# neuromodulation/PyPARRM

Measured on NVIDIA B200. Metric: filter_data channel-samples/sec, higher is better.
Workload: dtype f64

## Files before the change

### pyparrm_b200/_native.py

```python

from __future__ import annotations

import ctypes
import os
from ctypes import POINTER, c_char_p, c_double, c_int, c_int32, c_int64, c_size_t, c_void_p

LIB_NAME = "libparrm_b200.so"
LIB_PATH = os.path.join(os.path.dirname(os.path.abspath(__file__)), LIB_NAME)

F64, F32, I16, I32 = 0, 1, 2, 3
DIR_BOTH, DIR_PAST, DIR_FUTURE = 0, 1, 2
DIRECTIONS = {"both": DIR_BOTH, "past": DIR_PAST, "future": DIR_FUTURE}
MAX_BANDWIDTH = 23
NM_STATE_BYTES = 88
ABI_VERSION = 8
PLAN_AUTO, PLAN_GATHER, PLAN_COMB = 0, 1, 2
KERNEL_AUTO, KERNEL_GATHER, KERNEL_SPECIALISED = 0, 1, 3


class FilterOptions(ctypes.Structure):

    _fields_ = [
        ("kernel", c_int32),
        ("steps_per_chunk", c_int32),
# ... 112 lines not shown
            f"{LIB_NAME} is not built (expected {LIB_PATH}). Build it with "
            "`python -c 'import __graft_entry__ as g; g.build()'` or "
            "`pyparrm_b200/csrc/build.sh`. pyparrm_b200 has no CPU fallback."
        )
    lib = ctypes.CDLL(LIB_PATH)
    for name, (restype, argtypes) in SIGNATURES.items():
        fn = getattr(lib, name)
        fn.restype = restype
        fn.argtypes = argtypes
    if lib.parrm_abi_version() != ABI_VERSION:
        raise ImportError(
            f"{LIB_NAME} has ABI version {lib.parrm_abi_version()}, expected {ABI_VERSION}; rebuild it."
        )
    return lib


lib = _load()


def last_error() -> str:
    msg = lib.parrm_last_error()
    return msg.decode("utf-8", "replace") if msg else ""


def check(status: int, what: str) -> None:
    if status != 0:
        raise RuntimeError(f"{what} failed (status {status}): {last_error()}")


def filter_last_kernel() -> str:
    name = lib.parrm_filter_last_kernel()
    return name.decode() if name else ""


def device_count() -> int:
    return int(lib.parrm_device_count())


def plan_filter(taps, dtype: int = F64, strategy: int = PLAN_AUTO):
    import numpy as np

    taps = np.ascontiguousarray(taps, dtype=np.int32)
    nbytes = lib.parrm_filter_plan_bytes(taps.ctypes.data, int(taps.shape[0]))
    plan = np.zeros(nbytes, dtype=np.uint8)
    check(lib.parrm_filter_plan(taps.ctypes.data, int(taps.shape[0]), dtype, strategy,
                                plan.ctypes.data, nbytes), "parrm_filter_plan")
    info = np.zeros(16, dtype=np.int32)
    terms = np.zeros(256, dtype=np.int32)
    check(lib.parrm_filter_plan_info(plan.ctypes.data, info.ctypes.data, terms.ctypes.data, 256),
          "parrm_filter_plan_info")
    kind, stride, n_kinds, w0, w1, b0, b1, n_plus, n_minus, centre, cost = (int(v) for v in info[:11])
    cuts = np.cumsum([0, b0, b1, n_plus, n_minus])
    parts = [terms[cuts[i]:cuts[i + 1]].copy() for i in range(4)]
    desc = {
        "kind": kind, "stride": stride, "windows": [w0, w1][:n_kinds],
        "boxes": parts[:2][:n_kinds], "plus": parts[2], "minus": parts[3],
        "centre": centre, "cost": cost / 1000.0, "n_taps": int(info[11]),
    }
    return plan, desc
```

### pyparrm_b200/csrc/filter_comb_e.cuh

```cuda
#pragma once

#ifdef __CUDACC_RTC__
typedef signed char int8_t;
typedef int int32_t;
typedef unsigned int uint32_t;
typedef long long int64_t;
typedef unsigned long long uint64_t;
typedef unsigned long long uintptr_t;
#else
#include <stdint.h>
#endif

#ifndef PE_D
#define PE_T double
#define PE_D 200
#define PE_NK 2
#define PE_M0 20
#define PE_M1 10
#define PE_NB0 7
#define PE_NB1 2
#define PE_OFF0 -1969, -1954, -1923, -1877, -1846, -1831, -1800
#define PE_OFF1 -1908, 108
#define PE_NPLUS 1
#define PE_PLUS -2000
#define PE_NMINUS 0
#define PE_MINUS 0
#define PE_CENTRE -1
#define PE_U 10
#define PE_PF 2
#define PE_NTAPS 160
#define PE_WLO -2000
#define PE_WHI 2000
#define PE_BACK 108
#define PE_FWD 2000
#define PE_CTAS 2
#endif
#ifndef PE_VARIANT
#define PE_VARIANT 0
#endif

namespace parrm_e {

typedef PE_T T;
typedef double T2;
constexpr int D = PE_D;
constexpr int NK = PE_NK;
constexpr int M0 = PE_M0;
constexpr int M1 = PE_M1;
constexpr int NB0 = PE_NB0;
constexpr int NB1 = PE_NB1;
constexpr int NPLUS = PE_NPLUS;
constexpr int NMINUS = PE_NMINUS;
constexpr int CENTRE = PE_CENTRE;
constexpr int U = PE_U;
constexpr int PF = PE_PF;
constexpr int NTAPS = PE_NTAPS;
constexpr int WLO = PE_WLO;
constexpr int WHI = PE_WHI;
constexpr int BACK = PE_BACK;
constexpr int FWD = PE_FWD;
constexpr int ES = int(sizeof(T));
constexpr int VEC = 16 / ES;
constexpr int CH = U * D;
constexpr int HB = (BACK + CH - 1) / CH;
constexpr int HF = (FWD + CH - 1) / CH;
constexpr int MIR = HB + HF;
constexpr int Q = HB + HF + 1 + PF;
constexpr int GPB = (M0 + U - 1) / U;
constexpr int B = GPB * U;
constexpr int NPG = GPB;
constexpr int NW = (D + 31) / 32;
constexpr int NT = NW * 32 + 32;
constexpr int BAR_BYTES = ((2 * Q * 8 + 127) / 128) * 128;
constexpr int SMEM_BYTES = BAR_BYTES + (Q + MIR) * CH * ES;
static_assert((CH * ES) % 16 == 0, "chunk must be a whole number of 16-byte units");
static_assert(M0 >= M1 && M0 >= 1, "box lengths ordered");

__host__ __device__ constexpr int off0(int b) {
  constexpr int t[NB0 > 0 ? NB0 : 1] = {PE_OFF0};
  return t[b];
}
__host__ __device__ constexpr int off1(int b) {
  constexpr int t[NB1 > 0 ? NB1 : 1] = {PE_OFF1};
  return t[b];
}
__host__ __device__ constexpr int plus_tap(int i) {
  constexpr int t[NPLUS > 0 ? NPLUS : 1] = {PE_PLUS};
  return t[i];
}
__host__ __device__ constexpr int minus_tap(int i) {
  constexpr int t[NMINUS > 0 ? NMINUS : 1] = {PE_MINUS};
  return t[i];
}

struct Args {
  const T* x;
  T* out;
  const int32_t* taps;
  const int32_t* count;
  const T2* recip;
  int64_t ld_x, x_t0, n_x;
  int64_t ld_out, t0, n_out;
  int64_t n_total;
  int64_t total_groups;
  int32_t groups_per_chan;
  int32_t edge_start;
  int32_t edge_total;
  int32_t pad;
  unsigned long long* timeline;
  T neg_inv_n;
  T t_max;
};

__device__ __forceinline__ uint32_t smem_u32(const void* p) {
  return static_cast<uint32_t>(__cvta_generic_to_shared(p));
}
__device__ __forceinline__ void mbar_init(uint64_t* bar, uint32_t count) {
  asm volatile("mbarrier.init.shared::cta.b64 [%0], %1;" ::"r"(smem_u32(bar)), "r"(count));
}
__device__ __forceinline__ void mbar_expect_tx(uint64_t* bar, uint32_t bytes) {
  asm volatile("mbarrier.arrive.expect_tx.shared::cta.b64 _, [%0], %1;" ::"r"(smem_u32(bar)),
               "r"(bytes)
               : "memory");
}
__device__ __forceinline__ void mbar_arrive(uint64_t* bar) {
  asm volatile("mbarrier.arrive.shared::cta.b64 _, [%0];" ::"r"(smem_u32(bar)) : "memory");
}
__device__ __forceinline__ void mbar_wait(uint32_t bar, uint32_t parity) {
  asm volatile(
      "{\n"
      ".reg .pred p;\n"
      "WAIT_%=:\n"
      "mbarrier.try_wait.parity.shared::cta.b64 p, [%0], %1;\n"
      "@p bra DONE_%=;\n"
      "bra WAIT_%=;\n"
      "DONE_%=:\n"
      "}\n" ::"r"(bar),
      "r"(parity)
      : "memory");
}
__device__ __forceinline__ void bulk_g2s(void* dst_smem, const void* src_gmem, uint32_t bytes,
                                         uint64_t* bar) {
  asm volatile(
      "cp.async.bulk.shared::cluster.global.mbarrier::complete_tx::bytes [%0], [%1], %2, [%3];" ::
          "r"(smem_u32(dst_smem)),
      "l"(src_gmem), "r"(bytes), "r"(smem_u32(bar))
// ... 15 lines not shown
  const int n_in = count[v1 - (WLO - 1)] - count[v2 - (WLO - 1)];
  T y = xc - tot * T(recip[n_in]);
  if (n_in == 0) y = T(0);
  return y;
}

__device__ __noinline__ T direct_value(const int32_t* __restrict__ taps,
                                       const T2* __restrict__ recip, int64_t n_total, T t_max,
                                       const T* __restrict__ xrow, int64_t t, int64_t lo_valid,
                                       int64_t hi_valid) {
  T acc = T(0);
  int n_in = 0;
  for (int k = 0; k < NTAPS; ++k) {
    const int64_t g = t - taps[k];
    if (g < 0 || g >= n_total) continue;
    ++n_in;
    if (g >= lo_valid && g < hi_valid) acc += xrow[g];
  }
  if (n_in == 0) return T(0);
  const T y = xrow[t] - acc * T(recip[n_in]);
  return fabs(y) <= t_max ? y : T(0);
}

struct Walk {
  int pb;
  int rslot;
  int fslot;
  uint32_t fphase;
};

__device__ __forceinline__ void group_begin(Walk& w, uint32_t bars) {
  mbar_wait(bars + w.fslot * 8, w.fphase);
  if (++w.fslot == Q) {
    w.fslot = 0;
    w.fphase ^= 1u;
  }
}
__device__ __forceinline__ void group_end(Walk& w, uint32_t bars, int lane, unsigned wmask) {
  __syncwarp(wmask);
  if (lane == 0) {
    asm volatile("mbarrier.arrive.shared::cta.b64 _, [%0];" ::"r"(bars + (Q + w.rslot) * 8)
                 : "memory");
  }
  w.pb += CH * ES;
  if (++w.rslot == Q) {
    w.rslot = 0;
    w.pb -= Q * CH * ES;
  }
}

struct Rings {
  T r0[B];
  T r1[NK > 1 ? B : 1];
  T S0, S1;
};

__device__ __forceinline__ T ring_sum0(const Rings& r, int s) {
  T a = r.r0[s];
#pragma unroll
  for (int i = 1; i < M0; ++i) a += r.r0[(s + B - i) % B];
  return a;
}
__device__ __forceinline__ T ring_sum1(const Rings& r, int s) {
  if (NK < 2) return T(0);
  T a = r.r1[s];
#pragma unroll
  for (int i = 1; i < M1; ++i) a += r.r1[(s + B - i) % B];
  return a;
}

template <bool FAST>
__device__ __forceinline__ int run_block(Rings& r, Walk& w, const Args& a,
                                         const unsigned char* const smem, uint32_t bars,
                                         int lane, unsigned wmask, int c, T* const orow,
                                         int& bad_lo, int& bad_hi, int64_t Tb, int g,
                                         int n_groups) {
  const T neg_inv_n = a.neg_inv_n;
  const T t_max = a.t_max;
  T* const op = orow + Tb + c;
  int done = 0;
#pragma unroll
  for (int gi = 0; gi < GPB; ++gi) {
    if (!FAST && g + gi >= n_groups) break;
    group_begin(w, bars);
    int mode = 1;
    if (!FAST) {
      const int64_t Tn = Tb + int64_t(gi) * CH;
      const bool interior = (Tn - WHI >= 0) && (Tn + CH - WLO <= a.n_total);
      const bool all_out = (Tn >= a.t0) && (Tn + CH <= a.t0 + a.n_out);
      mode = (g + gi < NPG) ? 0 : ((interior && all_out) ? 1 : 2);
    }
    const unsigned char* const p = smem + w.pb;
#pragma unroll
    for (int js = 0; js < U; ++js) {
      const int s = gi * U + js;
      auto ld = [&](int off) {
        return *reinterpret_cast<const T*>(p + (HB * CH + js * D - off) * ES);
      };
      r.S0 -= r.r0[(s + B - M0) % B];
      if (NK > 1) r.S1 -= r.r1[(s + B - M1) % B];
      T e0 = ld(off0(0));
      if (NB0 > 1) {
        T e0b = ld(off0(1));
#pragma unroll
        for (int b = 2; b < NB0; ++b) {
          if (b & 1) e0b += ld(off0(b)); else e0 += ld(off0(b));
        }
        e0 += e0b;
      }
      r.r0[s] = e0;
      r.S0 += e0;
      T tot = r.S0;
      if (NK > 1) {
        T e1 = ld(off1(0));
        if (NB1 > 1) {
          T e1b = ld(off1(1));
#pragma unroll
          for (int b = 2; b < NB1; ++b) {
            if (b & 1) e1b += ld(off1(b)); else e1 += ld(off1(b));
          }
          e1 += e1b;
        }
        r.r1[s] = e1;
        r.S1 += e1;
        tot += r.S1;
      }
      T single = T(0);
      if (NPLUS > 0) {
        single = ld(plus_tap(0));
#pragma unroll
        for (int i = 1; i < NPLUS; ++i) single += ld(plus_tap(i));
      }
#pragma unroll
      for (int i = 0; i < NMINUS; ++i) single -= ld(minus_tap(i));
      const T xc = ld(0);
      if (CENTRE != 0) single = fma(T(CENTRE), xc, single);
      if (NPLUS > 0 || NMINUS > 0 || CENTRE != 0) tot += single;
      if (FAST) {
        T y = fma(tot, neg_inv_n, xc);
        if (__builtin_expect(!(fabs(y) <= t_max), 0)) {
          r.S0 = ring_sum0(r, s);
          r.S1 = ring_sum1(r, s);
          bad_lo = min(bad_lo, g * U + s);
          bad_hi = max(bad_hi, g * U + s);
          y = T(0);
        }
        op[s * D] = y;
      } else if (mode != 0) {
        const int64_t t = Tb + c + int64_t(s) * D;
        T y = mode == 1 ? fma(tot, neg_inv_n, xc) : edge_value(a.count, a.recip, t, a.n_total, xc, tot);
// ... 66 lines not shown
#if PE_VARIANT & 2
    ++tl_pieces;
#endif
    const int n_groups = NPG + int(n_end - n_first);
    const int n_chunks = n_groups + HB + HF;
    const int64_t c_first = n_first - NPG - HB;

    if (is_producer) {
      for (int i = 0; i < n_chunks; ++i) {
        const int64_t g0 = gamma + (c_first + i) * int64_t(CH);
        T* const dst = ring + fslot * CH;
        mbar_wait(bars + (Q + fslot) * 8, fphase ^ 1u);
        if (g0 >= lo_valid && g0 + CH <= hi_valid) {
          if (lane == 0) {
            asm volatile("fence.proxy.async.shared::cta;" ::: "memory");
            const bool mirror = fslot < MIR;
            mbar_expect_tx(&full[fslot], uint32_t(CH * ES) * (mirror ? 2u : 1u));
            bulk_g2s(dst, xrow + g0, uint32_t(CH * ES), &full[fslot]);
            if (mirror) bulk_g2s(dst + Q * CH, xrow + g0, uint32_t(CH * ES), &full[fslot]);
          }
        } else {
          for (int e = lane; e < CH; e += 32) {
            const int64_t g = g0 + e;
            const T v = (g >= lo_valid && g < hi_valid) ? xrow[g] : T(0);
            dst[e] = v;
            if (fslot < MIR) dst[Q * CH + e] = v;
          }
          __syncwarp();
          if (lane == 0) mbar_arrive(&full[fslot]);
        }
        if (++fslot == Q) {
          fslot = 0;
          fphase ^= 1u;
        }
      }
      continue;
    }

    if (tid >= D) continue;
    const int c = tid;
    const unsigned wmask = (tid | 31) < D ? 0xffffffffu : ((1u << (D & 31)) - 1u);
    for (int i = 0; i < HB + HF; ++i) {
      mbar_wait(bars + fslot * 8, fphase);
      if (++fslot == Q) {
        fslot = 0;
        fphase ^= 1u;
      }
    }
    Rings r;
#pragma unroll
    for (int s = 0; s < B; ++s) r.r0[s] = T(0);
#pragma unroll
    for (int s = 0; s < (NK > 1 ? B : 1); ++s) r.r1[s] = T(0);
    const int64_t T0 = gamma + (n_first - NPG) * int64_t(CH);
    Walk w;
    w.pb = BAR_BYTES + (rslot * CH + c) * ES;
    w.rslot = rslot;
    w.fslot = fslot;
    w.fphase = fphase;
    int bad_lo = 1 << 30, bad_hi = -1;
    for (int g = 0; g < n_groups;) {
      const int64_t Tb = T0 + int64_t(g) * CH;
      r.S0 = ring_sum0(r, B - 1);
      r.S1 = ring_sum1(r, B - 1);
      const bool fast = g >= NPG && g + GPB <= n_groups && Tb - WHI >= 0 &&
                        Tb + int64_t(B) * D - WLO <= a.n_total && Tb >= a.t0 &&
                        Tb + int64_t(B) * D <= a.t0 + a.n_out;
      if (fast) {
        g += run_block<true>(r, w, a, smem_raw, bars, lane, wmask, c, orow, bad_lo, bad_hi,
                             Tb, g, n_groups);
      } else {
        g += run_block<false>(r, w, a, smem_raw, bars, lane, wmask, c, orow, bad_lo, bad_hi,
                              Tb, g, n_groups);
      }
    }
    rslot = w.rslot;
    fslot = w.fslot;
    fphase = w.fphase;
    for (int k = bad_lo; k <= bad_hi; ++k) {
      const int64_t t = T0 + c + int64_t(k) * D;
      if (t >= a.t0 && t < a.t0 + a.n_out)
        orow[t] = direct_value(a.taps, a.recip, a.n_total, a.t_max, xrow, t, lo_valid, hi_valid);
    }
    __syncwarp(wmask);
    for (int i = 0; i < HB + HF; ++i) {
      if (lane == 0) mbar_arrive(&empty[rslot]);
      if (++rslot == Q) rslot = 0;
    }
  }
#if PE_VARIANT & 2
  if (tid == 0 && a.timeline) {
    unsigned long long tl_end;
    unsigned smid;
    asm volatile("mov.u64 %0, %%globaltimer;" : "=l"(tl_end));
    asm volatile("mov.u32 %0, %%smid;" : "=r"(smid));
    a.timeline[4 * blockIdx.x + 0] = smid;
    a.timeline[4 * blockIdx.x + 1] = tl_start;
    a.timeline[4 * blockIdx.x + 2] = tl_end;
    a.timeline[4 * blockIdx.x + 3] = tl_pieces;
  }
#endif
}

}
```

### pyparrm_b200/csrc/filter_jit.cu

```cuda
#include <cuda.h>
#include <dlfcn.h>
#include <string.h>

#include <algorithm>
#include <map>
#include <mutex>
#include <string>
#include <vector>

#include "common.cuh"
#include "filter_jit.h"
#include "filter_plan.h"

namespace parrm {
namespace {

const char kCombESource[] =
#include "filter_comb_e_src.inc"
    ;

typedef struct _nvrtcProgram* nvrtcProgram;
struct Nvrtc {
  void* handle = nullptr;
  int (*CreateProgram)(nvrtcProgram*, const char*, const char*, int, const char* const*,
                       const char* const*) = nullptr;
  int (*CompileProgram)(nvrtcProgram, int, const char* const*) = nullptr;
  int (*GetCUBINSize)(nvrtcProgram, size_t*) = nullptr;
  int (*GetCUBIN)(nvrtcProgram, char*) = nullptr;
  int (*GetProgramLogSize)(nvrtcProgram, size_t*) = nullptr;
  int (*GetProgramLog)(nvrtcProgram, char*) = nullptr;
  int (*DestroyProgram)(nvrtcProgram*) = nullptr;
  const char* (*GetErrorString)(int) = nullptr;
  bool ok = false;
};

Nvrtc* nvrtc() {
  static Nvrtc n;
  static std::once_flag once;
  std::call_once(once, [] {
    const char* names[] = {"libnvrtc.so.12", "libnvrtc.so", "/usr/local/cuda/lib64/libnvrtc.so.12",
                           "/usr/local/cuda/lib64/libnvrtc.so"};
    for (const char* name : names) {
      n.handle = dlopen(name, RTLD_NOW | RTLD_LOCAL);
      if (n.handle) break;
    }
    if (!n.handle) return;
#define PARRM_NVRTC_SYM(field, sym)                                             \
  n.field = reinterpret_cast<decltype(n.field)>(dlsym(n.handle, sym));          \
  if (!n.field) return;
    PARRM_NVRTC_SYM(CreateProgram, "nvrtcCreateProgram")
    PARRM_NVRTC_SYM(CompileProgram, "nvrtcCompileProgram")
    PARRM_NVRTC_SYM(GetCUBINSize, "nvrtcGetCUBINSize")
    PARRM_NVRTC_SYM(GetCUBIN, "nvrtcGetCUBIN")
    PARRM_NVRTC_SYM(GetProgramLogSize, "nvrtcGetProgramLogSize")
// ... 18 lines not shown
};

Driver* driver() {
  static Driver d;
  static std::once_flag once;
  std::call_once(once, [] {
    auto get = [](const char* name, void** fn) {
      cudaDriverEntryPointQueryResult st;
      return cudaGetDriverEntryPoint(name, fn, cudaEnableDefault, &st) == cudaSuccess &&
             st == cudaDriverEntryPointSuccess && *fn != nullptr;
    };
    d.ok = get("cuModuleLoadData", reinterpret_cast<void**>(&d.ModuleLoadData)) &&
           get("cuModuleGetFunction", reinterpret_cast<void**>(&d.ModuleGetFunction)) &&
           get("cuFuncSetAttribute", reinterpret_cast<void**>(&d.FuncSetAttribute)) &&
           get("cuFuncGetAttribute", reinterpret_cast<void**>(&d.FuncGetAttribute)) &&
           get("cuLaunchKernel", reinterpret_cast<void**>(&d.LaunchKernel)) &&
           get("cuGetErrorString", reinterpret_cast<void**>(&d.GetErrorString));
  });
  return &d;
}

int driver_fail(CUresult rc, const char* what) {
  const char* msg = nullptr;
  if (driver()->GetErrorString) driver()->GetErrorString(rc, &msg);
  set_error("%s: %s", what, msg ? msg : "driver error");
  return PARRM_ERR_CUDA;
}

struct Kernel {
  CUfunction fn = nullptr;
  int smem_bytes = 0, threads = 0, regs = 0, ctas_per_sm = 1;
  int chunk = 0, priming_groups = 0;
};

std::mutex g_mutex;
std::map<std::string, Kernel> g_cache;

std::string join(const int32_t* v, int n) {
  std::string s;
  for (int i = 0; i < n; ++i) {
    if (i) s += ",";
    s += std::to_string(v[i]);
  }
  if (n == 0) s = "0";
  return s;
}

}

bool comb_e_shape(const FilterPlanHeader* hdr, const int32_t* terms, int dtype,
                  const FilterTuning* tune, CombEShape* out) {
  const FilterPlanHeader* sec = hdr;
  if (hdr->kind != kPlanComb || sec->n_kinds < 1 || sec->n_kinds > 2) return false;
  CombEShape s;
  memset(&s, 0, sizeof(s));
  s.es = dtype == PARRM_F64 ? 8 : 4;
  s.d = sec->stride;
  s.nk = sec->n_kinds;
  const int nb[2] = {sec->n_box[0], sec->n_kinds > 1 ? sec->n_box[1] : 0};
  int first = 0;
  if (s.nk == 2 && sec->window[1] > sec->window[0]) first = 1;
  const int32_t* box[2] = {terms, terms + nb[0]};
  s.m[0] = sec->window[first];
  s.nb[0] = nb[first];
  s.off[0] = box[first];
  if (s.nk == 2) {
    s.m[1] = sec->window[1 - first];
    s.nb[1] = nb[1 - first];
    s.off[1] = box[1 - first];
  } else {
    s.m[1] = 1;
    s.nb[1] = 0;
    s.off[1] = nullptr;
  }
  s.n_plus = sec->n_plus;
  s.n_minus = sec->n_minus;
  s.plus = terms + nb[0] + nb[1];
  s.minus = s.plus + s.n_plus;
  s.centre = sec->centre;
  s.n_taps = hdr->n_taps;
  s.w_lo = hdr->w_min < 0 ? hdr->w_min : 0;
  s.w_hi = hdr->w_max > 0 ? hdr->w_max : 0;
  int lo = 0, hi = 0;
  const int n_all = nb[0] + nb[1] + s.n_plus + s.n_minus;
  for (int i = 0; i < n_all; ++i) {
    lo = terms[i] < lo ? terms[i] : lo;
    hi = terms[i] > hi ? terms[i] : hi;
  }
  s.back = hi;
  s.fwd = -lo;
  if (s.d < kPatternFirstMinStride || s.d > kPatternFirstMaxStride) return false;
  if (n_all > 96 || s.nb[0] < 1) return false;
  const int ring_regs = (s.m[0] + (s.nk > 1 ? s.m[1] : 0)) * (s.es / 4);
  const int threads = pattern_first_threads(s.d);
  auto reg_budget = [&](int ctas) { return pattern_first_reg_budget(s.d, ctas); };
  if (ring_regs + kPatternFirstStepRegs > reg_budget(1)) return false;
  int ctas_first = ring_regs + kPatternFirstStepRegs <= reg_budget(2) ? 2 : 1;
  if (s.es == 4 && 3 * threads <= 2048 && ring_regs + 40 <= reg_budget(3)) ctas_first = 3;
  if (tune && tune->ctas_per_sm > 0) ctas_first = tune->ctas_per_sm;
  const int pf_max = (tune && tune->prefetch_chunks > 0) ? tune->prefetch_chunks : 2;
  const int pf_min = std::min(pf_max, 2);
  auto smem_for = [&](int u, int pf) {
    const int64_t ch = int64_t(u) * s.d;
    const int64_t hb = (s.back + ch - 1) / ch, hf = (s.fwd + ch - 1) / ch;
    const int64_t q = hb + hf + 1 + pf;
    return ((2 * q * 8 + 127) / 128) * 128 + (q + hb + hf) * ch * s.es;
  };
  auto usable = [&](int u) {
    return u >= 1 && (int64_t(u) * s.d * s.es) % 16 == 0 && (s.m[0] + u - 1) / u * u <= 64;
  };
  for (int ctas = ctas_first; ctas >= 1; --ctas) {
    const int64_t budget = int64_t(227) * 1024 / ctas - 1024;
    int u = 0;
    if (tune && tune->steps_per_chunk > 0) {
      u = tune->steps_per_chunk;
      if (!usable(u) || smem_for(u, pf_min) > budget) u = 0;
    } else {
      for (int cand = s.m[0]; cand >= 1 && u == 0; --cand)
        if (s.m[0] % cand == 0 && int64_t(cand) * s.d * s.es <= 32768 &&
            int64_t(cand) * s.d >= 512 && usable(cand) && smem_for(cand, pf_min) <= budget)
          u = cand;
      const int u_hi = int(std::max<int64_t>(1, 20480 / (int64_t(s.d) * s.es)));
      for (int cand = u_hi; cand >= 1 && u == 0; --cand)
        if (usable(cand) && smem_for(cand, pf_min) <= budget) u = cand;
      for (int cand = 1; cand <= 64 && u == 0; ++cand)
        if (usable(cand) && smem_for(cand, pf_min) <= budget) u = cand;
    }
    if (u == 0) continue;
    int pf = pf_min;
    while (pf < pf_max && smem_for(u, pf + 1) <= budget) ++pf;
    s.smem_bytes = int(smem_for(u, pf));
    s.ctas = ctas;
    s.u = u;
    s.pf = pf;
    s.variant = tune ? tune->variant : 0;
    *out = s;
    return true;
  }
  return false;
}

static int compile_cubin(const CombEShape& s, std::vector<char>* cubin) {
  Nvrtc* n = nvrtc();
  if (!n->ok) {
    const char* why = dlerror();
    set_error("parrm filter: NVRTC (libnvrtc.so.12) could not be opened: %s", why ? why : "?");
    return PARRM_ERR_UNSUPPORTED;
  }
  std::vector<std::string> opts = {
      "--gpu-architecture=sm_100a", "-std=c++17", "-lineinfo",
      std::string("-DPE_T=") + (s.es == 8 ? "double" : "float"),
      "-DPE_D=" + std::to_string(s.d), "-DPE_NK=" + std::to_string(s.nk),
      "-DPE_M0=" + std::to_string(s.m[0]), "-DPE_M1=" + std::to_string(s.m[1]),
      "-DPE_NB0=" + std::to_string(s.nb[0]), "-DPE_NB1=" + std::to_string(s.nb[1]),
      "-DPE_OFF0=" + join(s.off[0], s.nb[0]), "-DPE_OFF1=" + join(s.off[1], s.nb[1]),
      "-DPE_NPLUS=" + std::to_string(s.n_plus), "-DPE_PLUS=" + join(s.plus, s.n_plus),
      "-DPE_NMINUS=" + std::to_string(s.n_minus), "-DPE_MINUS=" + join(s.minus, s.n_minus),
      "-DPE_CENTRE=" + std::to_string(s.centre), "-DPE_U=" + std::to_string(s.u),
      "-DPE_PF=" + std::to_string(s.pf), "-DPE_NTAPS=" + std::to_string(s.n_taps),
      "-DPE_WLO=" + std::to_string(s.w_lo), "-DPE_WHI=" + std::to_string(s.w_hi),
      "-DPE_BACK=" + std::to_string(s.back), "-DPE_FWD=" + std::to_string(s.fwd),
      "-DPE_CTAS=" + std::to_string(s.ctas), "-DPE_VARIANT=" + std::to_string(s.variant)};
  std::vector<const char*> copts;
  for (const std::string& o : opts) copts.push_back(o.c_str());
  nvrtcProgram prog = nullptr;
  int rc = n->CreateProgram(&prog, kCombESource, "filter_comb_e.cu", 0, nullptr, nullptr);
  if (rc != 0) {
    set_error("nvrtcCreateProgram: %s", n->GetErrorString(rc));
    return PARRM_ERR_CUDA;
  }
  rc = n->CompileProgram(prog, int(copts.size()), copts.data());
  if (rc != 0) {
    size_t log_size = 0;
    n->GetProgramLogSize(prog, &log_size);
    std::string log(log_size + 1, '\0');
    if (log_size) n->GetProgramLog(prog, &log[0]);
    set_error("nvrtcCompileProgram: %s\n%.380s", n->GetErrorString(rc), log.c_str());
    n->DestroyProgram(&prog);
    return PARRM_ERR_CUDA;
  }
  size_t cubin_size = 0;
  n->GetCUBINSize(prog, &cubin_size);
  cubin->resize(cubin_size);
  rc = n->GetCUBIN(prog, cubin->data());
  n->DestroyProgram(&prog);
  if (rc != 0 || cubin_size == 0) {
    set_error("nvrtcGetCUBIN: %s", n->GetErrorString(rc));
    return PARRM_ERR_CUDA;
  }
  return PARRM_OK;
}

int comb_e_compile_only(const CombEShape& s, size_t* cubin_bytes) {
  std::vector<char> cubin;
  const int rc = compile_cubin(s, &cubin);
  if (rc == PARRM_OK && cubin_bytes) *cubin_bytes = cubin.size();
  return rc;
}

static int build_kernel(const CombEShape& s, Kernel* out) {
  Driver* d = driver();
  if (!d->ok) {
    set_error("parrm filter: CUDA driver entry points unavailable");
    return PARRM_ERR_UNSUPPORTED;
  }
  std::vector<char> cubin;
  const int rc = compile_cubin(s, &cubin);
  if (rc != PARRM_OK) return rc;
  PARRM_CUDA_OK(cudaFree(nullptr));
  CUmodule mod = nullptr;
  CUresult cr = d->ModuleLoadData(&mod, cubin.data());
  if (cr != CUDA_SUCCESS) return driver_fail(cr, "cuModuleLoadData");
  Kernel k;
  cr = d->ModuleGetFunction(&k.fn, mod, "parrm_filter_comb_e");
  if (cr != CUDA_SUCCESS) return driver_fail(cr, "cuModuleGetFunction");
  k.smem_bytes = s.smem_bytes;
  k.threads = ((s.d + 31) / 32) * 32 + 32;
  k.ctas_per_sm = s.ctas;
  k.chunk = s.u * s.d;
  k.priming_groups = (s.m[0] + s.u - 1) / s.u;
  cr = d->FuncSetAttribute(k.fn, CU_FUNC_ATTRIBUTE_MAX_DYNAMIC_SHARED_SIZE_BYTES, k.smem_bytes);
  if (cr != CUDA_SUCCESS) return driver_fail(cr, "cuFuncSetAttribute(max dynamic shared memory)");
  d->FuncSetAttribute(k.fn, CU_FUNC_ATTRIBUTE_PREFERRED_SHARED_MEMORY_CARVEOUT, 100);
  d->FuncGetAttribute(&k.regs, CU_FUNC_ATTRIBUTE_NUM_REGS, k.fn);
  *out = k;
  return PARRM_OK;
}

bool comb_e_cached(const CombEShape& s) {
  int dev = 0;
  if (cudaGetDevice(&dev) != cudaSuccess) return false;
  const std::string key = comb_e_key(s, dev);
  std::lock_guard<std::mutex> lock(g_mutex);
  return g_cache.count(key) != 0;
}

std::string comb_e_key(const CombEShape& s, int dev) {
  std::string key = std::to_string(dev) + "|" + std::to_string(s.es) + "|" + std::to_string(s.d) +
                    "|" + std::to_string(s.nk) + "|" + std::to_string(s.m[0]) + "|" +
                    std::to_string(s.m[1]) + "|" + join(s.off[0], s.nb[0]) + "|" +
                    join(s.off[1], s.nb[1]) + "|" + join(s.plus, s.n_plus) + "|" +
                    join(s.minus, s.n_minus) + "|" + std::to_string(s.centre) + "|" +
                    std::to_string(s.u) + "|" + std::to_string(s.pf) + "|" +
                    std::to_string(s.n_taps) + "|" + std::to_string(s.w_lo) + "|" +
                    std::to_string(s.w_hi) + "|" + std::to_string(s.ctas) + "|" +
                    std::to_string(s.variant);
  return key;
}

int launch_comb_e(const CombEShape& s, const void* d_x, void* d_out, const int32_t* d_taps,
                  const int32_t* d_count, const double* d_recip,
                  int64_t ld_x, int64_t x_t0, int64_t n_x, int64_t ld_out, int64_t t0,
                  int64_t n_out, int64_t n_total, int64_t n_chans, cudaStream_t stream,
                  int* regs_out, unsigned long long timeline) {
  int dev = 0;
  PARRM_CUDA_OK(cudaGetDevice(&dev));
  const std::string key = comb_e_key(s, dev);
  Kernel k;
  {
    std::lock_guard<std::mutex> lock(g_mutex);
    auto it = g_cache.find(key);
    if (it == g_cache.end()) {
      const int rc = build_kernel(s, &k);
      if (rc != PARRM_OK) return rc;
      g_cache[key] = k;
    } else {
      k = it->second;
    }
  }
  if (regs_out) *regs_out = k.regs;
  struct Args {
    const void* x;
    void* out;
    const int32_t* taps;
    const int32_t* count;
    const double* recip;
    int64_t ld_x, x_t0, n_x, ld_out, t0, n_out, n_total, total_groups;
    int32_t groups_per_chan, edge_start, edge_total, pad;
    unsigned long long timeline;
    unsigned char consts[16];
  } a;
  a.x = d_x; a.out = d_out; a.taps = d_taps; a.count = d_count; a.recip = d_recip;
  a.ld_x = ld_x; a.x_t0 = x_t0; a.n_x = n_x;
  a.ld_out = ld_out; a.t0 = t0; a.n_out = n_out; a.n_total = n_total;
  const int64_t ch = k.chunk;
  a.groups_per_chan = int32_t(ceil_div(n_out + ch - 1, ch));
  const int gpb = k.priming_groups;
  const int edge_end = 2 * gpb;
  a.edge_start = s.variant & 4 ? 0 : 2 * gpb + 2 + edge_end;
  a.edge_total = s.variant & 4 ? 0 : a.edge_start + edge_end;
  a.total_groups = n_chans * int64_t(a.groups_per_chan + a.edge_total);
  a.pad = 0;
  a.timeline = timeline;
  memset(a.consts, 0, sizeof(a.consts));
  if (s.es == 8) {
    const double v[2] = {-1.0 / double(s.n_taps), 1.7976931348623157e308};
    memcpy(a.consts, v, sizeof(v));
  } else {
    const float v[2] = {-1.0f / float(s.n_taps), 3.402823466e38f};
// ... 15 lines not shown
```

### pyparrm_b200/csrc/filter_jit.h

```cpp
#pragma once
#include <cuda_runtime.h>
#include <stdint.h>

#include <string>

#include "filter_plan.h"

namespace parrm {

struct FilterTuning {
  int kernel;
  int steps_per_chunk;
  int prefetch_chunks;
  int ctas_per_sm;
  int variant;
  unsigned long long timeline;
};

struct CombEShape {
  int es;
  int d, nk, m[2], nb[2];
  const int32_t* off[2];
  int n_plus, n_minus;
  const int32_t *plus, *minus;
  int centre, n_taps, w_lo, w_hi, back, fwd;
  int u, pf, ctas, smem_bytes, variant;
};

bool comb_e_shape(const FilterPlanHeader* hdr, const int32_t* terms, int dtype,
                  const FilterTuning* tune, CombEShape* out);
std::string comb_e_key(const CombEShape& s, int dev);
bool comb_e_cached(const CombEShape& s);
int comb_e_compile_only(const CombEShape& s, size_t* cubin_bytes);
int launch_comb_e(const CombEShape& s, const void* d_x, void* d_out, const int32_t* d_taps,
                  const int32_t* d_count, const double* d_recip,
                  int64_t ld_x, int64_t x_t0, int64_t n_x, int64_t ld_out, int64_t t0,
                  int64_t n_out, int64_t n_total, int64_t n_chans, cudaStream_t stream,
                  int* regs_out, unsigned long long timeline = 0);

}
```

### pyparrm_b200/csrc/filter_plan.cu

```cuda
#include <algorithm>
#include <string.h>
#include <vector>

#include "common.cuh"
#include "filter_plan.h"

namespace parrm {
namespace {

struct CombPlan {
  int d = 0, nk = 0;
  int m[kMaxBoxKinds] = {0, 0};
  std::vector<int> box[kMaxBoxKinds];
  std::vector<int> plus, minus;
  int centre = 0;
  double cost = 1e30;
  int n_terms() const { return int(box[0].size() + box[1].size() + plus.size() + minus.size()); }
};

bool cover(const std::vector<uint8_t>& bit, int lo, int hi, int d, int nk, const int* m,
           CombPlan* out) {
  const int span = hi - lo + 1;
  CombPlan p;
  p.d = d;
  p.nk = nk;
  for (int k = 0; k < nk; ++k) p.m[k] = m[k];
  std::vector<int> dp, zeros, choice;
  for (int c = 0; c < d && c < span; ++c) {
    const int len = (span - 1 - c) / d + 1;
    dp.assign(len + 1, 0);
    zeros.assign(len + 1, 0);
    choice.assign(len + 1, -1);
    auto w_of = [&](int pos) { return lo + c + pos * d; };
    for (int q = 0; q < len; ++q) {
      const int w = w_of(q);
      const bool free_zero = (w == 0);
      zeros[q + 1] = zeros[q] + ((bit[w - lo] == 0 && !free_zero) ? 1 : 0);
    }
    const int kInf = 1 << 28;
    for (int q = 1; q <= len; ++q) dp[q] = kInf;
    for (int q = 0; q < len; ++q) {
      if (dp[q] >= kInf) continue;
      const int single = dp[q] + (bit[w_of(q) - lo] ? 1 : 0);
      if (single < dp[q + 1]) {
        dp[q + 1] = single;
        choice[q + 1] = -1;
      }
      for (int k = 0; k < nk; ++k) {
        if (q + m[k] > len) continue;
        const int v = dp[q] + 1 + (zeros[q + m[k]] - zeros[q]);
        if (v < dp[q + m[k]]) {
          dp[q + m[k]] = v;
          choice[q + m[k]] = k;
// ... 80 lines not shown
      };
      for (int64_t w = lo; w <= hi; ++w) {
        if (!has(w) || has(w - d)) continue;
        int len = 1;
        while (has(w + int64_t(len) * d)) ++len;
        if (len < 2) continue;
        bool seen = false;
        for (auto& e : lengths)
          if (e.second == len) {
            e.first += len;
            seen = true;
          }
        if (!seen) lengths.emplace_back(len, len);
      }
    }
    std::sort(lengths.rbegin(), lengths.rend());
    const int max_ring = pattern_first_max_ring(d, es);
    if (max_ring < 2) continue;
    std::vector<int> cand;
    auto add_len = [&](int len) {
      if (len >= 2 && len <= max_ring && std::find(cand.begin(), cand.end(), len) == cand.end())
        cand.push_back(len);
    };
    for (size_t i = 0; i < lengths.size() && i < 6; ++i) add_len(lengths[i].second);
    for (size_t i = 0; i < lengths.size() && i < 3 && cand.size() < 8; ++i) {
      const int len = lengths[i].second;
      if (len > max_ring || 2 * len > max_ring) {
        add_len((len + 1) / 2);
        add_len((len + 2) / 3);
      }
    }
    const int n_len = int(cand.size());
    for (int i = 0; i < n_len; ++i) {
      for (int j = i; j < n_len; ++j) {
        int m[2] = {cand[i], cand[j]};
        if (i != j && m[0] + m[1] > max_ring) continue;
        CombPlan p;
        if (!cover(bit, lo, hi, d, i == j ? 1 : 2, m, &p)) continue;
        if (p.n_terms() > kMaxTerms) continue;
        const int ring = p.m[0] + (p.nk > 1 ? p.m[1] : 0);
        if (ring > max_ring) continue;
        p.cost = double(p.n_terms()) + 1e-3 * ring;
        if (p.cost < best->cost) {
          *best = p;
          found = true;
        }
      }
    }
  }
  if (!found) return false;
  return exact(*best, bit, lo, hi);
}

}
}

extern "C" {

static size_t plan_layout(const int32_t* h_taps, int32_t n_taps, size_t* recip_off, size_t* count_off) {
  const size_t n = size_t(n_taps > 0 ? n_taps : 0);
  size_t off = sizeof(parrm::FilterPlanHeader) + (n + parrm::kMaxTerms) * sizeof(int32_t);
  off = (off + 7) & ~size_t(7);
  if (recip_off) *recip_off = off;
  off += (n + 1) * sizeof(double);
  if (count_off) *count_off = off;
  int64_t span = 0;
  if (n > 0 && h_taps != nullptr) {
    const int64_t lo = h_taps[0] < 0 ? h_taps[0] : 0;
    const int64_t hi = h_taps[n - 1] > 0 ? h_taps[n - 1] : 0;
    span = hi - lo;
  }
  off += size_t(span + 2) * sizeof(int32_t);
  return (off + 15) & ~size_t(15);
}

size_t parrm_filter_plan_bytes(const int32_t* h_taps, int32_t n_taps) {
  return plan_layout(h_taps, n_taps, nullptr, nullptr);
}

int parrm_filter_plan(const int32_t* h_taps, int32_t n_taps, int dtype, int strategy,
                      void* h_plan, size_t plan_bytes) {
  using namespace parrm;
  PARRM_REQUIRE(n_taps > 0 && h_taps != nullptr, "parrm_filter_plan: empty tap list");
  PARRM_REQUIRE(h_plan != nullptr, "parrm_filter_plan: null plan buffer");
  PARRM_REQUIRE(dtype == PARRM_F64 || dtype == PARRM_F32, "parrm_filter_plan: bad dtype");
  PARRM_REQUIRE(strategy >= PARRM_PLAN_AUTO && strategy <= PARRM_PLAN_COMB,
                "parrm_filter_plan: unknown strategy %d", strategy);
  for (int32_t i = 1; i < n_taps; ++i)
    PARRM_REQUIRE(h_taps[i] > h_taps[i - 1], "parrm_filter_plan: taps must be strictly ascending");
  PARRM_REQUIRE(h_taps[0] > -(1 << 30) && h_taps[n_taps - 1] < (1 << 30),
                "parrm_filter_plan: tap offset out of range");
  size_t recip_off = 0, count_off = 0;
  const size_t total = plan_layout(h_taps, n_taps, &recip_off, &count_off);
  PARRM_REQUIRE(plan_bytes >= total, "parrm_filter_plan: plan buffer too small (%zu < %zu)",
                plan_bytes, total);
  PARRM_REQUIRE(total < (size_t(1) << 31), "parrm_filter_plan: tap window too wide");
  memset(h_plan, 0, total);
  FilterPlanHeader* hdr = static_cast<FilterPlanHeader*>(h_plan);
  hdr->magic = kPlanMagic;
  hdr->version = kPlanVersion;
  hdr->n_taps = n_taps;
  hdr->w_min = h_taps[0];
  hdr->w_max = h_taps[n_taps - 1];
  hdr->kind = kPlanGather;
  hdr->taps_offset = int32_t(sizeof(FilterPlanHeader));
  hdr->dtype = dtype;
  hdr->terms_offset = hdr->taps_offset + n_taps * int32_t(sizeof(int32_t));
  hdr->cost_milli = n_taps * 1000;
  unsigned char* base = static_cast<unsigned char*>(h_plan);
  memcpy(base + hdr->taps_offset, h_taps, size_t(n_taps) * sizeof(int32_t));
  {
    hdr->recip_offset = int32_t(recip_off);
    hdr->count_offset = int32_t(count_off);
    hdr->total_bytes = int32_t(total);
    double* recip = reinterpret_cast<double*>(base + recip_off);
    recip[0] = 0.0;
    for (int32_t i = 1; i <= n_taps; ++i) recip[i] = 1.0 / double(i);
    int32_t* count = reinterpret_cast<int32_t*>(base + count_off);
    const int64_t w_lo = h_taps[0] < 0 ? h_taps[0] : 0;
    const int64_t w_hi = h_taps[n_taps - 1] > 0 ? h_taps[n_taps - 1] : 0;
    int32_t i = 0;
    for (int64_t v = w_lo - 1; v <= w_hi; ++v) {
      while (i < n_taps && h_taps[i] <= v) ++i;
      count[v - (w_lo - 1)] = i;
    }
  }
  if (strategy == PARRM_PLAN_GATHER) return PARRM_OK;

  CombPlan best;
  const bool ok = best_comb(h_taps, n_taps, kPatternFirstMinStride, kPatternFirstMaxStride,
                            dtype == PARRM_F64 ? 8 : 4, &best);
  const bool worth = ok && (strategy == PARRM_PLAN_COMB || best.cost < 0.6 * double(n_taps));
  if (!worth) {
    if (strategy == PARRM_PLAN_COMB) {
      set_error("parrm_filter_plan: this tap set has no comb structure");
      return PARRM_ERR_UNSUPPORTED;
    }
    return PARRM_OK;
  }
  hdr->kind = kPlanComb;
  hdr->stride = best.d;
  hdr->n_kinds = best.nk;
  int32_t* terms = reinterpret_cast<int32_t*>(base + hdr->terms_offset);
  int n = 0;
  for (int k = 0; k < best.nk; ++k) {
    hdr->window[k] = best.m[k];
    hdr->n_box[k] = int32_t(best.box[k].size());
    hdr->a_min[k] = best.box[k].front();
    hdr->a_max[k] = best.box[k].back();
    for (int a : best.box[k]) terms[n++] = a;
  }
  hdr->n_plus = int32_t(best.plus.size());
  hdr->n_minus = int32_t(best.minus.size());
  for (int w : best.plus) terms[n++] = w;
  for (int w : best.minus) terms[n++] = w;
  hdr->centre = best.centre;
  hdr->cost_milli = int32_t(best.cost * 1000.0);
  return PARRM_OK;
}

}

extern "C" int parrm_filter_plan_info(const void* h_plan, int32_t* info, int32_t* terms,
                                      int32_t capacity) {
  using namespace parrm;
  PARRM_REQUIRE(h_plan != nullptr && info != nullptr, "parrm_filter_plan_info: null pointer");
  const FilterPlanHeader* hdr = static_cast<const FilterPlanHeader*>(h_plan);
  PARRM_REQUIRE(hdr->magic == kPlanMagic && hdr->version == kPlanVersion,
                "parrm_filter_plan_info: not a filter plan");
  const int32_t n_terms = hdr->kind == kPlanComb
                              ? hdr->n_box[0] + hdr->n_box[1] + hdr->n_plus + hdr->n_minus
                              : 0;
  const int32_t v[16] = {hdr->kind, hdr->stride, hdr->n_kinds, hdr->window[0], hdr->window[1],
                         hdr->n_box[0], hdr->n_box[1], hdr->n_plus, hdr->n_minus, hdr->centre,
                         hdr->cost_milli, hdr->n_taps, hdr->w_min, hdr->w_max, n_terms, 0};
  for (int i = 0; i < 16; ++i) info[i] = v[i];
  if (terms != nullptr) {
    PARRM_REQUIRE(capacity >= n_terms, "parrm_filter_plan_info: terms buffer too small");
    const int32_t* src = reinterpret_cast<const int32_t*>(
        static_cast<const unsigned char*>(h_plan) + hdr->terms_offset);
    for (int i = 0; i < n_terms; ++i) terms[i] = src[i];
  }
  return PARRM_OK;
}
```

### pyparrm_b200/csrc/filter_plan.h

```cpp
#pragma once
#include <stdint.h>

namespace parrm {

constexpr uint32_t kPlanMagic = 0x4D525250u;
constexpr uint32_t kPlanVersion = 4;
constexpr int kMaxTerms = 120;
constexpr int kMaxBoxKinds = 2;

enum PlanKind : int32_t {
  kPlanGather = 0,
  kPlanComb = 1
};

struct FilterPlanHeader {
  uint32_t magic;
  uint32_t version;
  int32_t n_taps;
  int32_t w_min, w_max;
  int32_t kind;
  int32_t taps_offset;
  int32_t dtype;
  int32_t stride;
  int32_t n_kinds;
  int32_t window[kMaxBoxKinds];
  int32_t n_box[kMaxBoxKinds];
  int32_t a_min[kMaxBoxKinds];
  int32_t a_max[kMaxBoxKinds];
  int32_t n_plus, n_minus;
  int32_t centre;
  int32_t terms_offset;
  int32_t cost_milli;
  int32_t count_offset;
  int32_t recip_offset;
  int32_t total_bytes;
  int32_t reserved[6];
};
static_assert(sizeof(FilterPlanHeader) == 128, "plan header is 128 bytes");

constexpr int kPatternFirstMinStride = 64;
constexpr int kPatternFirstMaxStride = 992;
constexpr int kPatternFirstMaxRing = 60;
constexpr int kPatternFirstStepRegs = 52;

inline int pattern_first_threads(int d) { return ((d + 31) / 32) * 32 + 32; }
inline int pattern_first_reg_budget(int d, int ctas) {
  const int r = (65536 / (ctas * pattern_first_threads(d))) / 8 * 8;
  return r < 255 ? r : 255;
}
inline int pattern_first_max_ring(int d, int es) {
  const int ring = (pattern_first_reg_budget(d, 1) - kPatternFirstStepRegs) / (es / 4);
  return ring < kPatternFirstMaxRing ? ring : kPatternFirstMaxRing;
}

}
```

Before: 308.4 billion.

## Serve comb tap loads from register delay lines instead of re-reading memory

The planner now finds pairs of comb load offsets that differ by a multiple of the stride and records them as reuse entries. The JIT kernel keeps per-entry register delay lines so that one offset's load is satisfied by a value loaded several steps earlier, cutting shared-memory traffic. Reuse entries are sized to fit the spare register budget. The JIT compiles with ptxas verbose output, counts spill bytes, and drops reuse entries until spills do not exceed the plain build. The cost is extra registers, multiple NVRTC compiles per shape, and a plan format version bump.

```diff
diff --git a/pyparrm_b200/_native.py b/pyparrm_b200/_native.py
--- a/pyparrm_b200/_native.py
+++ b/pyparrm_b200/_native.py
@@ -188,9 +188,11 @@
     kind, stride, n_kinds, w0, w1, b0, b1, n_plus, n_minus, centre, cost = (int(v) for v in info[:11])
     cuts = np.cumsum([0, b0, b1, n_plus, n_minus])
     parts = [terms[cuts[i]:cuts[i + 1]].copy() for i in range(4)]
+    reuse = terms[cuts[4]:cuts[4] + 3 * int(info[15])].reshape(-1, 3)
     desc = {
         "kind": kind, "stride": stride, "windows": [w0, w1][:n_kinds],
         "boxes": parts[:2][:n_kinds], "plus": parts[2], "minus": parts[3],
         "centre": centre, "cost": cost / 1000.0, "n_taps": int(info[11]),
+        "reuse": [tuple(int(v) for v in r) for r in reuse],
     }
     return plan, desc
diff --git a/pyparrm_b200/csrc/filter_comb_e.cuh b/pyparrm_b200/csrc/filter_comb_e.cuh
--- a/pyparrm_b200/csrc/filter_comb_e.cuh
+++ b/pyparrm_b200/csrc/filter_comb_e.cuh
@@ -34,6 +34,8 @@
 #define PE_BACK 108
 #define PE_FWD 2000
 #define PE_CTAS 2
+#define PE_NREUSE 1
+#define PE_REUSE -1800, -2000, 1
 #endif
 #ifndef PE_VARIANT
 #define PE_VARIANT 0
@@ -59,6 +61,7 @@
 constexpr int WHI = PE_WHI;
 constexpr int BACK = PE_BACK;
 constexpr int FWD = PE_FWD;
+constexpr int NR = (PE_VARIANT & 8) ? 0 : PE_NREUSE;
 constexpr int ES = int(sizeof(T));
 constexpr int VEC = 16 / ES;
 constexpr int CH = U * D;
@@ -92,6 +95,17 @@
   constexpr int t[NMINUS > 0 ? NMINUS : 1] = {PE_MINUS};
   return t[i];
 }
+
+__host__ __device__ constexpr int reuse(int i, int f) {
+  constexpr int t[PE_NREUSE > 0 ? 3 * PE_NREUSE : 3] = {PE_REUSE};
+  return t[3 * i + f];
+}
+__host__ __device__ constexpr int served_by(int off) {
+  for (int i = 0; i < NR; ++i)
+    if (reuse(i, 0) == off) return i;
+  return -1;
+}
+static_assert(NR == 0 || (reuse(0, 2) >= 1 && reuse(0, 2) <= B), "delay within one block");
 
 struct Args {
   const T* x;
@@ -213,6 +227,7 @@
 struct Rings {
   T r0[B];
   T r1[NK > 1 ? B : 1];
+  T dl[NR > 0 ? NR : 1][B];
   T S0, S1;
 };
 
@@ -255,8 +270,20 @@
 #pragma unroll
     for (int js = 0; js < U; ++js) {
       const int s = gi * U + js;
+      T served[NR > 0 ? NR : 1];
+#pragma unroll
+      for (int i = 0; i < NR; ++i) served[i] = r.dl[i][(s + B - reuse(i, 2)) % B];
       auto ld = [&](int off) {
-        return *reinterpret_cast<const T*>(p + (HB * CH + js * D - off) * ES);
+        const int i = served_by(off);
+        T v;
+        if (i >= 0 && (FAST || s >= reuse(i, 2) || g != 0))
+          v = served[i];
+        else
+          v = *reinterpret_cast<const T*>(p + (HB * CH + js * D - off) * ES);
+#pragma unroll
+        for (int j = 0; j < NR; ++j)
+          if (reuse(j, 1) == off) r.dl[j][s] = v;
+        return v;
       };
       r.S0 -= r.r0[(s + B - M0) % B];
       if (NK > 1) r.S1 -= r.r1[(s + B - M1) % B];
@@ -429,6 +456,10 @@
     for (int s = 0; s < B; ++s) r.r0[s] = T(0);
 #pragma unroll
     for (int s = 0; s < (NK > 1 ? B : 1); ++s) r.r1[s] = T(0);
+#pragma unroll
+    for (int i = 0; i < NR; ++i)
+#pragma unroll
+      for (int s = 0; s < B; ++s) r.dl[i][s] = T(0);
     const int64_t T0 = gamma + (n_first - NPG) * int64_t(CH);
     Walk w;
     w.pb = BAR_BYTES + (rslot * CH + c) * ES;
diff --git a/pyparrm_b200/csrc/filter_jit.cu b/pyparrm_b200/csrc/filter_jit.cu
--- a/pyparrm_b200/csrc/filter_jit.cu
+++ b/pyparrm_b200/csrc/filter_jit.cu
@@ -1,5 +1,6 @@
 #include <cuda.h>
 #include <dlfcn.h>
+#include <stdio.h>
 #include <string.h>
 
 #include <algorithm>
@@ -124,6 +125,9 @@
                   const FilterTuning* tune, CombEShape* out) {
   const FilterPlanHeader* sec = hdr;
   if (hdr->kind != kPlanComb || sec->n_kinds < 1 || sec->n_kinds > 2) return false;
+  const int32_t* reuse = reinterpret_cast<const int32_t*>(
+      reinterpret_cast<const unsigned char*>(hdr) + hdr->reuse_offset);
+  const int n_reuse = hdr->n_reuse;
   CombEShape s;
   memset(&s, 0, sizeof(s));
   s.es = dtype == PARRM_F64 ? 8 : 4;
@@ -203,6 +207,8 @@
     while (pf < pf_max && smem_for(u, pf + 1) <= budget) ++pf;
     s.smem_bytes = int(smem_for(u, pf));
     s.ctas = ctas;
+    s.n_reuse = n_reuse;
+    s.reuse = reuse;
     s.u = u;
     s.pf = pf;
     s.variant = tune ? tune->variant : 0;
@@ -212,7 +218,19 @@
   return false;
 }
 
-static int compile_cubin(const CombEShape& s, std::vector<char>* cubin) {
+static int spill_bytes(const std::string& log) {
+  int total = 0;
+  for (size_t p = log.find("stack frame, "); p != std::string::npos;
+       p = log.find("stack frame, ", p + 1)) {
+    int st = 0, ld = 0;
+    if (sscanf(log.c_str() + p, "stack frame, %d bytes spill stores, %d bytes spill loads", &st,
+               &ld) == 2)
+      total += st + ld;
+  }
+  return total;
+}
+
+static int compile_cubin(const CombEShape& s, std::vector<char>* cubin, int* spills) {
   Nvrtc* n = nvrtc();
   if (!n->ok) {
     const char* why = dlerror();
@@ -232,7 +250,9 @@
       "-DPE_PF=" + std::to_string(s.pf), "-DPE_NTAPS=" + std::to_string(s.n_taps),
       "-DPE_WLO=" + std::to_string(s.w_lo), "-DPE_WHI=" + std::to_string(s.w_hi),
       "-DPE_BACK=" + std::to_string(s.back), "-DPE_FWD=" + std::to_string(s.fwd),
-      "-DPE_CTAS=" + std::to_string(s.ctas), "-DPE_VARIANT=" + std::to_string(s.variant)};
+      "-DPE_CTAS=" + std::to_string(s.ctas), "-DPE_VARIANT=" + std::to_string(s.variant),
+      "-DPE_NREUSE=" + std::to_string(s.n_reuse), "-DPE_REUSE=" + join(s.reuse, 3 * s.n_reuse)};
+  if (spills) opts.push_back("--ptxas-options=-v");
   std::vector<const char*> copts;
   for (const std::string& o : opts) copts.push_back(o.c_str());
   nvrtcProgram prog = nullptr;
@@ -251,6 +271,13 @@
     n->DestroyProgram(&prog);
     return PARRM_ERR_CUDA;
   }
+  if (spills) {
+    size_t log_size = 0;
+    n->GetProgramLogSize(prog, &log_size);
+    std::string log(log_size + 1, '\0');
+    if (log_size) n->GetProgramLog(prog, &log[0]);
+    *spills = spill_bytes(log);
+  }
   size_t cubin_size = 0;
   n->GetCUBINSize(prog, &cubin_size);
   cubin->resize(cubin_size);
@@ -263,9 +290,27 @@
   return PARRM_OK;
 }
 
+static int compile_settled(CombEShape s, std::vector<char>* cubin) {
+  if (s.n_reuse == 0 || (s.variant & 8)) return compile_cubin(s, cubin, nullptr);
+  CombEShape none = s;
+  none.n_reuse = 0;
+  std::vector<char> plain;
+  int spill_none = 0;
+  int rc = compile_cubin(none, &plain, &spill_none);
+  if (rc != PARRM_OK) return rc;
+  for (; s.n_reuse > 0; --s.n_reuse) {
+    int spill = 0;
+    rc = compile_cubin(s, cubin, &spill);
+    if (rc != PARRM_OK) return rc;
+    if (spill <= spill_none) return PARRM_OK;
+  }
+  cubin->swap(plain);
+  return PARRM_OK;
+}
+
 int comb_e_compile_only(const CombEShape& s, size_t* cubin_bytes) {
   std::vector<char> cubin;
-  const int rc = compile_cubin(s, &cubin);
+  const int rc = compile_settled(s, &cubin);
   if (rc == PARRM_OK && cubin_bytes) *cubin_bytes = cubin.size();
   return rc;
 }
@@ -277,7 +322,7 @@
     return PARRM_ERR_UNSUPPORTED;
   }
   std::vector<char> cubin;
-  const int rc = compile_cubin(s, &cubin);
+  const int rc = compile_settled(s, &cubin);
   if (rc != PARRM_OK) return rc;
   PARRM_CUDA_OK(cudaFree(nullptr));
   CUmodule mod = nullptr;
@@ -316,7 +361,7 @@
                     std::to_string(s.u) + "|" + std::to_string(s.pf) + "|" +
                     std::to_string(s.n_taps) + "|" + std::to_string(s.w_lo) + "|" +
                     std::to_string(s.w_hi) + "|" + std::to_string(s.ctas) + "|" +
-                    std::to_string(s.variant);
+                    std::to_string(s.variant) + "|" + join(s.reuse, 3 * s.n_reuse);
   return key;
 }
 
diff --git a/pyparrm_b200/csrc/filter_jit.h b/pyparrm_b200/csrc/filter_jit.h
--- a/pyparrm_b200/csrc/filter_jit.h
+++ b/pyparrm_b200/csrc/filter_jit.h
@@ -24,6 +24,8 @@
   int n_plus, n_minus;
   const int32_t *plus, *minus;
   int centre, n_taps, w_lo, w_hi, back, fwd;
+  int n_reuse;
+  const int32_t* reuse;
   int u, pf, ctas, smem_bytes, variant;
 };
 
diff --git a/pyparrm_b200/csrc/filter_plan.cu b/pyparrm_b200/csrc/filter_plan.cu
--- a/pyparrm_b200/csrc/filter_plan.cu
+++ b/pyparrm_b200/csrc/filter_plan.cu
@@ -1,4 +1,5 @@
 #include <algorithm>
+#include <array>
 #include <string.h>
 #include <vector>
 
@@ -185,6 +186,32 @@
   return exact(*best, bit, lo, hi);
 }
 
+std::vector<std::array<int, 3>> choose_reuse(const CombPlan& p, int budget) {
+  std::vector<int> loads = {0};
+  for (int k = 0; k < p.nk; ++k) loads.insert(loads.end(), p.box[k].begin(), p.box[k].end());
+  loads.insert(loads.end(), p.plus.begin(), p.plus.end());
+  loads.insert(loads.end(), p.minus.begin(), p.minus.end());
+  std::sort(loads.begin(), loads.end());
+  loads.erase(std::unique(loads.begin(), loads.end()), loads.end());
+  const int depth = std::max(p.m[0], p.nk > 1 ? p.m[1] : 0);
+  std::vector<std::array<int, 3>> cand;
+  for (int dst : loads)
+    for (int k = 1; k <= depth; ++k)
+      if (std::binary_search(loads.begin(), loads.end(), dst - k * p.d)) {
+        cand.push_back({k, dst, dst - k * p.d});
+        break;
+      }
+  std::sort(cand.begin(), cand.end());
+  std::vector<std::array<int, 3>> out;
+  int used = 0;
+  for (const auto& c : cand) {
+    if (used + c[0] > budget || int(out.size()) == kMaxReuse) break;
+    used += c[0];
+    out.push_back({c[1], c[2], c[0]});
+  }
+  return out;
+}
+
 }
 }
 
@@ -192,7 +219,8 @@
 
 static size_t plan_layout(const int32_t* h_taps, int32_t n_taps, size_t* recip_off, size_t* count_off) {
   const size_t n = size_t(n_taps > 0 ? n_taps : 0);
-  size_t off = sizeof(parrm::FilterPlanHeader) + (n + parrm::kMaxTerms) * sizeof(int32_t);
+  size_t off = sizeof(parrm::FilterPlanHeader) +
+               (n + parrm::kMaxTerms + 3 * parrm::kMaxReuse) * sizeof(int32_t);
   off = (off + 7) & ~size_t(7);
   if (recip_off) *recip_off = off;
   off += (n + 1) * sizeof(double);
@@ -239,6 +267,7 @@
   hdr->taps_offset = int32_t(sizeof(FilterPlanHeader));
   hdr->dtype = dtype;
   hdr->terms_offset = hdr->taps_offset + n_taps * int32_t(sizeof(int32_t));
+  hdr->reuse_offset = hdr->terms_offset + kMaxTerms * int32_t(sizeof(int32_t));
   hdr->cost_milli = n_taps * 1000;
   unsigned char* base = static_cast<unsigned char*>(h_plan);
   memcpy(base + hdr->taps_offset, h_taps, size_t(n_taps) * sizeof(int32_t));
@@ -289,6 +318,13 @@
   for (int w : best.minus) terms[n++] = w;
   hdr->centre = best.centre;
   hdr->cost_milli = int32_t(best.cost * 1000.0);
+  const int es = dtype == PARRM_F64 ? 8 : 4;
+  const int ring = best.m[0] + (best.nk > 1 ? best.m[1] : 0);
+  const auto reuse = choose_reuse(best, pattern_first_delay_budget(best.d, es, ring));
+  hdr->n_reuse = int32_t(reuse.size());
+  int32_t* rt = reinterpret_cast<int32_t*>(base + hdr->reuse_offset);
+  for (size_t i = 0; i < reuse.size(); ++i)
+    for (int f = 0; f < 3; ++f) rt[3 * i + f] = reuse[i][f];
   return PARRM_OK;
 }
 
@@ -306,13 +342,17 @@
                               : 0;
   const int32_t v[16] = {hdr->kind, hdr->stride, hdr->n_kinds, hdr->window[0], hdr->window[1],
                          hdr->n_box[0], hdr->n_box[1], hdr->n_plus, hdr->n_minus, hdr->centre,
-                         hdr->cost_milli, hdr->n_taps, hdr->w_min, hdr->w_max, n_terms, 0};
+                         hdr->cost_milli, hdr->n_taps, hdr->w_min, hdr->w_max, n_terms,
+                         hdr->kind == kPlanComb ? hdr->n_reuse : 0};
   for (int i = 0; i < 16; ++i) info[i] = v[i];
   if (terms != nullptr) {
-    PARRM_REQUIRE(capacity >= n_terms, "parrm_filter_plan_info: terms buffer too small");
-    const int32_t* src = reinterpret_cast<const int32_t*>(
-        static_cast<const unsigned char*>(h_plan) + hdr->terms_offset);
+    const int32_t n_out = n_terms + 3 * v[15];
+    PARRM_REQUIRE(capacity >= n_out, "parrm_filter_plan_info: terms buffer too small");
+    const unsigned char* base = static_cast<const unsigned char*>(h_plan);
+    const int32_t* src = reinterpret_cast<const int32_t*>(base + hdr->terms_offset);
     for (int i = 0; i < n_terms; ++i) terms[i] = src[i];
+    const int32_t* rt = reinterpret_cast<const int32_t*>(base + hdr->reuse_offset);
+    for (int i = 0; i < 3 * v[15]; ++i) terms[n_terms + i] = rt[i];
   }
   return PARRM_OK;
 }
diff --git a/pyparrm_b200/csrc/filter_plan.h b/pyparrm_b200/csrc/filter_plan.h
--- a/pyparrm_b200/csrc/filter_plan.h
+++ b/pyparrm_b200/csrc/filter_plan.h
@@ -4,9 +4,10 @@
 namespace parrm {
 
 constexpr uint32_t kPlanMagic = 0x4D525250u;
-constexpr uint32_t kPlanVersion = 4;
+constexpr uint32_t kPlanVersion = 5;
 constexpr int kMaxTerms = 120;
 constexpr int kMaxBoxKinds = 2;
+constexpr int kMaxReuse = 8;
 
 enum PlanKind : int32_t {
   kPlanGather = 0,
@@ -34,7 +35,9 @@
   int32_t count_offset;
   int32_t recip_offset;
   int32_t total_bytes;
-  int32_t reserved[6];
+  int32_t n_reuse;
+  int32_t reuse_offset;
+  int32_t reserved[4];
 };
 static_assert(sizeof(FilterPlanHeader) == 128, "plan header is 128 bytes");
 
@@ -53,4 +56,9 @@
   return ring < kPatternFirstMaxRing ? ring : kPatternFirstMaxRing;
 }
 
+inline int pattern_first_delay_budget(int d, int es, int ring) {
+  const int v = (pattern_first_reg_budget(d, 1) - kPatternFirstStepRegs) / (es / 4) - ring;
+  return v > 0 ? v : 0;
 }
+
+}
```

After: 309.3 billion, median of 6. About the same (+0.3%).
